# jason2714/de-i2i-gan

Measured on AMD Instinct MI355X. Metric: paired 256x256 images/sec (G+D train step), higher is better.
Workload: dtype bf16

## Files before the change

de-i2i-gan_amd/_lib.py:

```python
import ctypes
import os
from ctypes import POINTER, Structure, c_char_p, c_double, c_float, c_int, c_int64, c_size_t, c_void_p

_HERE = os.path.dirname(os.path.abspath(__file__))
LIB_PATH = os.path.join(_HERE, "lib", "libdei2i_hip.so")

BF16, F32 = 0, 1
ACT_NONE, ACT_RELU, ACT_LRELU = 0, 1, 2
PAD_ZERO, PAD_REFLECT = 0, 1
PROF_GATHER_GEMM, PROF_WGRAD, PROF_HALO_CONV, PROF_HALO_FOLD = 0, 1, 2, 3


class ConvDesc(Structure):
    _fields_ = [("dtype", c_int), ("N", c_int), ("H", c_int), ("W", c_int), ("Cin", c_int), ("Cout", c_int),
                ("CinS", c_int), ("CoutS", c_int), ("kh", c_int), ("kw", c_int), ("stride", c_int), ("pad", c_int),
                ("pad_mode", c_int), ("up", c_int)]


class ProDesc(Structure):
    _fields_ = [("A", c_void_p), ("B", c_void_p), ("n_stride", c_int), ("slope", c_float), ("ring", c_void_p)]


class EpiNormDesc(Structure):
    _fields_ = [("kind", c_int), ("up", c_int), ("act", c_int), ("group_images", c_int), ("x", c_void_p), ("mean", c_void_p),
# ... 86 lines not shown
    "dei2i_diffaug": (c_int, [c_int, c_int, c_int, c_int, c_int, c_int, c_int, c_int, _P, _P, _P, _P, _P]),
    "dei2i_prof_enable": (c_int, [c_int, c_int]),
    "dei2i_prof_collect": (c_int, [c_int, POINTER(c_int64), POINTER(c_double), POINTER(c_double)]),
    "dei2i_prof_collect_timed": (c_int, [c_int, POINTER(c_int64), POINTER(c_double)]),
    "dei2i_conv2d_fused_supported": (c_int, [_CD, c_int]),
    "dei2i_conv2d_stats_chunks": (c_int, [_CD]),
    "dei2i_conv2d_fwd_fused": (c_int, [_CD, _P, _P, _P, c_int, _P, _PD, _P, _P]),
    "dei2i_conv2d_wgrad_pro_supported": (c_int, [_CD]),
    "dei2i_conv2d_wgrad_oihw_pro": (c_int, [_CD, _P, _P, _P, c_size_t, _P, c_int, _PD, _P]),
    "dei2i_ring_pixels": (c_size_t, [c_int, c_int]),
    "dei2i_conv2d_ring_supported": (c_int, [_CD]),
    "dei2i_conv2d_dgrad_norm_supported": (c_int, [_CD]),
    "dei2i_conv2d_dgrad_norm_chunks": (c_int, [_CD]),
    "dei2i_conv2d_dgrad_input_norm": (c_int, [_CD, _P, _P, _P, _ED, _P]),
    "dei2i_in_act_bwd": (c_int, [c_int, c_int, c_int, c_int, c_int, _P, _P, _P, _P, c_float, _P, _P, _P, _P, _P, _P]),
    "dei2i_in_affine_act_bwd": (c_int, [c_int, c_int, c_int, c_int, c_int, _P, _P, _P, _P, c_float, _P, _P, _P, _P, _P, _P, _P]),
    "dei2i_avgpool2_fwd": (c_int, [c_int, c_int, c_int, c_int, c_int, _P, _P, _P]),
    "dei2i_avgpool2_bwd": (c_int, [c_int, c_int, c_int, c_int, c_int, _P, _P, _P]),
    "dei2i_spade_bwd_border": (c_int, [c_int, c_int, c_int, c_int, c_int, c_int, _P, _P, _P, _P, _P, _P, _P]),
    "dei2i_conv2d_fwd_ring": (c_int, [_CD, _P, _P, _P, _P, c_int, _P, _P, _P]),
    "dei2i_affine_act_img_fwd": (c_int, [c_int, c_int, c_int, c_int, _P, _P, _P, c_float, _P, _P]),
    "dei2i_spade_prep": (c_int, [c_int, c_int, c_int, c_int, c_int, c_int, _P, _P, c_int, c_float, _P, _P, _P, _P, _P, _P, _P]),
    "dei2i_affine_act_stats_fwd": (c_int, [c_int, c_int, c_int, c_int, c_int, _P, _P, _P, _P, c_int, _P, _P, _P]),
    "dei2i_launch_counts": (c_int, [POINTER(c_int64), c_int]),
    "dei2i_launch_counts_reset": (None, []),
    "dei2i_kernel_name": (c_char_p, [c_int]),
}

_lib = None


def load():
    global _lib
    if _lib is not None:
        return _lib
    import torch
    path = os.environ.get("DEI2I_LIB", LIB_PATH)
    if not os.path.exists(path):
        raise RuntimeError(
            f"libdei2i_hip.so not found at {path}: build it with `python -c 'import __graft_entry__ as g; g.build()'` "
            "(hipcc --offload-arch=gfx950).  There is no CPU / PyTorch fallback for the de-i2i-gan_amd ops.")
    lib = ctypes.CDLL(path)
    for name, (res, args) in SIGNATURES.items():
        fn = getattr(lib, name)
        fn.restype = res
        fn.argtypes = args
# ... 19 lines not shown
```

de-i2i-gan_amd/csrc/conv_api.hip:

```cpp
#include <hip/hip_runtime.h>

#include "../../include/dei2i_hip.h"
#include "launch.h"

namespace dei2i {

int g_use_wgrad_v2 = 1;
int g_use_wgrad_halo = 1;
int g_use_wgrad_thin = 1;
int g_dgrad_s2_ring = 1;
extern int g_halo16, g_halo16_fold;

static ConvShape to_shape(const dei2i_conv* c) {
  ConvShape s;
  s.N = c->N; s.H = c->H; s.W = c->W; s.Cin = c->Cin; s.Cout = c->Cout;
  s.kh = c->kh; s.kw = c->kw; s.stride = c->stride; s.pad = c->pad; s.pad_mode = c->pad_mode; s.up = c->up;
  return s;
}

static bool valid_conv(const dei2i_conv* c) {
  if (!c) return false;
  const int vec = c->dtype == DT_BF16 ? 8 : 4;
  if (c->dtype != DT_BF16 && c->dtype != DT_F32) return false;
  if (c->N <= 0 || c->H <= 0 || c->W <= 0 || c->Cin <= 0 || c->Cout <= 0) return false;
  if (c->CinS < c->Cin || c->CoutS < c->Cout || c->CinS % vec || c->CoutS % vec) return false;
  if (c->kh <= 0 || c->kw <= 0 || c->stride <= 0 || c->pad < 0 || c->up < 0 || c->up > 1) return false;
  if (c->kh < c->stride || c->kw < c->stride) return false;
  if (c->pad_mode == PAD_REFLECT && (c->pad >= (c->H << c->up) || c->pad >= (c->W << c->up))) return false;
  if (((c->H << c->up) + 2 * c->pad) < c->kh || ((c->W << c->up) + 2 * c->pad) < c->kw) return false;
  return true;
}

template <typename T>
// ... 74 lines not shown
    const int co = co0 + col, ci = ci0 + ch * VEC;
    if (co >= Cout || ci >= CinS) continue;
    float v[VEC];
#pragma unroll
    for (int e = 0; e < VEC; ++e) v[e] = tile[r * PT_ROW + ch * VEC + e];
    *reinterpret_cast<u32x4*>(fwd + ((size_t)co * taps + t) * CinS + ci) = Elem<T>::pack(v);
  }
  constexpr int DCH = PT_CO / VEC;
  for (int k = 0; k < pa.ncls; ++k) {
    const int th = pa.th[k], tw = pa.tw[k], nt = th * tw;
    T* dst = dgrad + pa.cls_begin[k];
    for (int i = threadIdx.x; i < PT_CI * nt * DCH; i += 256) {
      const int ch = i % DCH, r = i / DCH;
      const int t = r % nt, cil = r / nt;
      const int ci = ci0 + cil, co = co0 + ch * VEC;
      if (ci >= Cin || co >= CoutS) continue;
      const int jy = t / tw, jx = t - jy * tw;
      const int tap = (pa.ay[k] + s * jy) * kw + (pa.ax[k] + s * jx);
      float v[VEC];
#pragma unroll
      for (int e = 0; e < VEC; ++e) v[e] = tile[((ch * VEC + e) * taps + tap) * PT_ROW + cil];
      *reinterpret_cast<u32x4*>(dst + ((size_t)ci * nt + t) * CoutS + co) = Elem<T>::pack(v);
    }
  }
}

template <typename T>
__global__ void fold_pad_kernel(const T* __restrict__ ext, const T* __restrict__ addend, T* __restrict__ dx, int N, int H,
                                int W, int C, int pad, int reflect, int up) {
  constexpr int VEC = Elem<T>::VEC;
  const int Hl = H << up, Wl = W << up;
  const int off = reflect ? pad : 0;
  const int OH = Hl + 2 * off, OW = Wl + 2 * off;
  const int cv = C / VEC;
  const size_t total = (size_t)N * H * W * cv;
  for (size_t i = (size_t)blockIdx.x * blockDim.x + threadIdx.x; i < total; i += (size_t)gridDim.x * blockDim.x) {
    const int c = (int)(i % cv) * VEC;
    size_t r = i / cv;
    const int w = (int)(r % W); r /= W;
    const int h = (int)(r % H);
    const int n = (int)(r / H);
    float acc[VEC];
#pragma unroll
    for (int e = 0; e < VEC; ++e) acc[e] = 0.f;
    if (addend != nullptr) {
      float t[VEC];
// ... 272 lines not shown
    e = gather_gemm_multi(c->dtype, rows, wrows4, 4, dy, wd_packed, c->Cin, nullptr, ext_scratch, ws, ws_bytes, c->CinS, ACT_NONE, st, true);
    if (e != hipSuccess) return (int)e;
    const GatherDesc cols[4] = {sub_rect_desc(fr[0][0], 1, fr[0][0].Ho - 1, 0, 1), sub_rect_desc(fr[1][0], 0, fr[1][0].Ho - 1, 0, 1),
                                sub_rect_desc(fr[0][1], 1, fr[0][1].Ho - 1, fr[0][1].Wo - 1, 1),
                                sub_rect_desc(fr[1][1], 0, fr[1][1].Ho - 1, fr[1][1].Wo - 1, 1)};
    const long long wcols4[4] = {woff[0][0], woff[1][0], woff[0][1], woff[1][1]};
    e = gather_gemm_multi(c->dtype, cols, wcols4, 4, dy, wd_packed, c->Cin, nullptr, ext_scratch, ws, ws_bytes, c->CinS, ACT_NONE, st, true);
    if (e != hipSuccess) return (int)e;
    const int vec = c->dtype == DT_BF16 ? 8 : 4;
    const size_t total = (size_t)c->N * (2 * c->W + 2 * (c->H - 2)) * (c->CinS / vec);
    if (c->dtype == DT_BF16)
      hipLaunchKernelGGL(fold_border_kernel<bf16_t>, dim3(grid_for(total, 256)), dim3(256), 0, st, (const bf16_t*)ext_scratch, (bf16_t*)dx,
                         c->N, c->H, c->W, c->CinS, 1);
    else
      hipLaunchKernelGGL(fold_border_kernel<float>, dim3(grid_for(total, 256)), dim3(256), 0, st, (const float*)ext_scratch, (float*)dx, c->N,
                         c->H, c->W, c->CinS, 1);
    return (int)hipGetLastError();
  }
  const int rc = dei2i_conv2d_dgrad(c, dy, wd_packed, ext_scratch, ws, ws_bytes, s);
  if (rc != 0) return rc;
  return dei2i_fold_pad(c->dtype, c->N, c->H, c->W, c->CinS, c->pad, c->pad_mode, c->up, ext_scratch, nullptr, dx, s);
}

static bool dgrad_norm_shape_ok(const dei2i_conv* c) {
  if (!g_halo16 || !g_halo16_fold) return false;
  if (!valid_conv(c) || c->dtype != DT_BF16 || c->up) return false;
  if (c->kh != 3 || c->kw != 3 || c->stride != 1 || c->pad != 1 || c->pad_mode != PAD_REFLECT) return false;
  if (c->H % 16 != 0 || c->W % 32 != 0 || c->H < 32 || c->W < 64 || c->CinS < 64 || c->CinS % 8 != 0 || c->CoutS % 32 != 0) return false;
  if ((long long)c->N * c->H * c->W * c->CoutS >= (1ll << 31)) return false;
  const int tiles_m = c->N * (c->H / 16) * (c->W / 32);
  const int tn = c->CinS >= 128 ? (c->CinS + 127) / 128 : 1;
  return tiles_m * tn >= (num_cu() * 7) / 8;
}

int dei2i_conv2d_dgrad_norm_supported(const dei2i_conv* c) { return dgrad_norm_shape_ok(c) ? 1 : 0; }

int dei2i_conv2d_dgrad_norm_chunks(const dei2i_conv* c) { return (c->H / 16) * (c->W / 32); }

int dei2i_conv2d_dgrad_input_norm(const dei2i_conv* c, const void* dy, const void* wd_packed, void* dx, const dei2i_epi_norm* en,
                                  dei2i_stream s) {
  if (!dy || !wd_packed || !dx || !en || !dgrad_norm_shape_ok(c)) return DEI2I_ERR_BAD_ARG;
  if (!en->x || !en->mean || !en->rstd || !en->partial || en->up < 0 || en->up > 1) return DEI2I_ERR_BAD_ARG;
  const int kind = en->kind;
  if (kind == 1 ? !en->gb : (kind != 2 || !en->a || !en->b || en->up)) return DEI2I_ERR_BAD_ARG;
  if (en->group_images < 0 || (en->group_images > 0 && c->N % en->group_images != 0)) return DEI2I_ERR_BAD_ARG;
  ConvShape sh = to_shape(c);
// ... 151 lines not shown
```

de-i2i-gan_amd/csrc/geom.h:

```cpp
#pragma once
#include "common.h"

namespace dei2i {

struct GatherDesc {
  int N, Hs, Ws, Cs;
  int Clog;
  int Hl, Wl, up;
  int Ho, Wo, M;
  int sh, sw, by0, bx0;
  int th, tw, ys, xs;
  int pad_mode;
  int K;
  int wK, wtw, wty0, wtx0;
  int OH, OW, oys, oxs, oy0, ox0;
  int out_identity;
  FastDiv fd_cs, fd_tw, fd_wo, fd_howo;
};

inline void finish_desc(GatherDesc& g) {
  g.Hl = g.Hs << g.up;
  g.Wl = g.Ws << g.up;
  g.M = g.N * g.Ho * g.Wo;
  g.K = g.th * g.tw * g.Cs;
// ... 159 lines not shown
  int up;
  int act;
  int group_images;
};

DEI2I_HD long long packed_fwd_src(long long i, int Cin, int CinS, int taps) {
  const int ci = (int)(i % CinS);
  const long long r = i / CinS;
  const int t = (int)(r % taps);
  const long long co = r / taps;
  return ci < Cin ? (co * Cin + ci) * taps + t : -1;
}

DEI2I_HD long long packed_dgrad_src(long long i, int Cout, int Cin, int CoutS, int kh, int kw, int s, int ay, int ax,
                                    int th, int tw) {
  const int co = (int)(i % CoutS);
  const long long r = i / CoutS;
  const int t = (int)(r % (th * tw));
  const long long ci = r / (th * tw);
  const int jy = t / tw, jx = t - jy * tw;
  return co < Cout ? (((long long)co * Cin + ci) * kh + (ay + s * jy)) * kw + (ax + s * jx) : -1;
}

DEI2I_HD int fold_sources(int hs, int up, int Hl, int pad, int reflect, int* out) {
  const int off = reflect ? pad : 0;
  int n = 0;
  for (int a = 0; a < (1 << up); ++a) {
    const int hl = (hs << up) + a;
    out[n++] = hl + off;
    if (reflect) {
      if (hl >= 1 && hl <= pad) out[n++] = pad - hl;
      if (hl >= Hl - 1 - pad && hl <= Hl - 2) out[n++] = 2 * (Hl - 1) - hl + pad;
    }
  }
  return n;
}

}
```

de-i2i-gan_amd/csrc/reduce.hip:

```cpp
#include <hip/hip_runtime.h>
#include <math.h>

#include "../../include/dei2i_hip.h"
#include "launch.h"

namespace dei2i {

static inline int vec_of(int dtype) { return dtype == DT_BF16 ? 8 : 4; }

template <int NV, int VEC, typename OT = float>
DEI2I_D void block_combine_store(const float (&vals)[NV][VEC], int cv, int rpp, float* smem, OT* __restrict__ dst, int C) {
  const int tid = threadIdx.x;
  const int vcol = tid % cv, prow = tid / cv;
  __syncthreads();
  if (prow < rpp) {
#pragma unroll
    for (int q = 0; q < NV; ++q)
#pragma unroll
      for (int e = 0; e < VEC; ++e) smem[((q * VEC + e) * rpp + prow) * cv + vcol] = vals[q][e];
  }
  __syncthreads();
#pragma unroll 1
  for (int o = tid; o < NV * VEC * cv; o += 256) {
    const int qe = o / cv, vc = o - qe * cv;
// ... 311 lines not shown
        db[e] = g;
        v[0][e] += dxh;
        v[1][e] = fmaf(dxh, xh, v[1][e]);
      }
      if (gb_mode == 0) {
        *reinterpret_cast<u32x4*>(dgb_dense + q.opix * 2 * C + c) = Elem<T>::pack(dg);
        *reinterpret_cast<u32x4*>(dgb_dense + q.opix * 2 * C + C + c) = Elem<T>::pack(db);
      } else if (q.interior) {
#pragma unroll
        for (int e = 0; e < VEC; ++e) { v[2][e] += dg[e]; v[3][e] += db[e]; }
      }
    };
    int r = rbeg + prow;
    for (; r + rpp < rend; r += 2 * rpp) {
      const Row q0 = load(r), q1 = load(r + rpp);
      use(q0); use(q1);
    }
    if (r < rend) use(load(r));
  }
  block_combine_store<4, VEC>(v, cv, rpp, smem, partial + ((size_t)n * chunks + chunk) * 4 * C, C);
}

template <typename T>
__global__ __launch_bounds__(256) void spade_bwd_border_kernel(const T* __restrict__ dz, const T* __restrict__ x,
                                                               const float* __restrict__ mean, const float* __restrict__ rstd,
                                                               const T* __restrict__ gb, T* __restrict__ dgb_cls, int H,
                                                               int W, int C, int up, float slope = 0.f) {
  constexpr int VEC = Elem<T>::VEC;
  extern __shared__ float smem[];
  const int cls = blockIdx.x, n = blockIdx.y;
  const int cy = cls / 5, cx = cls - cy * 5;
  if (cy == 2 && cx == 2) return;
  const int cv = C / VEC, rpp = 256 / cv;
  const int tid = threadIdx.x, vcol = tid % cv, prow = tid / cv;
  const int Hs = H >> up, Ws = W >> up;
  const int y0 = cy < 2 ? cy : (cy == 2 ? 2 : H - 5 + cy), ny = cy == 2 ? H - 4 : 1;
  const int x0 = cx < 2 ? cx : (cx == 2 ? 2 : W - 5 + cx), nx = cx == 2 ? W - 4 : 1;
  const int count = ny * nx;
  float v[2][VEC];
#pragma unroll
  for (int e = 0; e < VEC; ++e) v[0][e] = v[1][e] = 0.f;
  if (prow < rpp) {
    const int c = vcol * VEC;
    float mv[VEC], rv[VEC], gm[VEC], bt[VEC];
    ldcoef<VEC>(mean + (size_t)n * C + c, mv);
    ldcoef<VEC>(rstd + (size_t)n * C + c, rv);
    const size_t gpix = ((size_t)n * 5 + cy) * 5 + cx;
    Elem<T>::unpack(*reinterpret_cast<const u32x4*>(gb + gpix * 2 * C + c), gm);
    Elem<T>::unpack(*reinterpret_cast<const u32x4*>(gb + gpix * 2 * C + C + c), bt);
    for (int i = prow; i < count; i += rpp) {
      const int h = y0 + i / nx, w = x0 + i % nx;
      const size_t opix = ((size_t)n * H + h) * W + w;
      float d[VEC], xv[VEC];
      Elem<T>::unpack(*reinterpret_cast<const u32x4*>(dz + opix * C + c), d);
      Elem<T>::unpack(*reinterpret_cast<const u32x4*>(x + (((size_t)n * Hs + (h >> up)) * Ws + (w >> up)) * C + c), xv);
#pragma unroll
      for (int e = 0; e < VEC; ++e) {
        const float xh = (xv[e] - mv[e]) * rv[e];
        const float g = fmaf(xh, 1.f + gm[e], bt[e]) > 0.f ? d[e] : slope * d[e];
        v[0][e] = fmaf(g, xh, v[0][e]);
        v[1][e] += g;
      }
    }
  }
  block_combine_store<2, VEC, T>(v, cv, rpp, smem, dgb_cls + (((size_t)n * 5 + cy) * 5 + cx) * 2 * C, C);
}

__global__ __launch_bounds__(256) void spade_bwd_finalize_kernel(const float* __restrict__ partial, int N, int chunks, int C,
                                                                 double count, float* __restrict__ coef,
                                                                 void* __restrict__ dgb_cls, int dtype) {
  const int c = blockIdx.x, n = blockIdx.y;
  double sq[4];
  combine_records<4>(partial, (size_t)n * chunks, chunks, C, c, sq);
  if (threadIdx.x != 0) return;
  coef[((size_t)n * 2 + 0) * C + c] = (float)(sq[0] / count);
  coef[((size_t)n * 2 + 1) * C + c] = (float)(sq[1] / count);
  if (dgb_cls != nullptr) {
// ... 34 lines not shown
    for (int e = 0; e < VEC; ++e) { acc[e] = 0.f; xh[e] = (xv[e] - mv[e]) * rv[e]; }
    for (int a = 0; a < (1 << up); ++a)
      for (int b = 0; b < (1 << up); ++b) {
        const int h = (hs << up) + a, w = (ws << up) + b;
        const size_t opix = ((size_t)n * H + h) * W + w;
        const size_t gpix = gb_mode == 0 ? opix : ((size_t)n * 5 + border_class(h, H)) * 5 + border_class(w, W);
        float d[VEC], gm[VEC], bt[VEC];
        Elem<T>::unpack(*reinterpret_cast<const u32x4*>(dz + opix * C + c), d);
        Elem<T>::unpack(*reinterpret_cast<const u32x4*>(gb + gpix * 2 * C + c), gm);
        Elem<T>::unpack(*reinterpret_cast<const u32x4*>(gb + gpix * 2 * C + C + c), bt);
#pragma unroll
        for (int e = 0; e < VEC; ++e) {
          const float g = fmaf(xh[e], 1.f + gm[e], bt[e]) > 0.f ? d[e] : slope * d[e];
          acc[e] = fmaf(g, 1.f + gm[e], acc[e]);
        }
      }
    float ad[VEC];
    if (addend != nullptr) Elem<T>::unpack(*reinterpret_cast<const u32x4*>(addend + i * VEC), ad);
    ldcoef<VEC>(coef + ((size_t)n * 2) * C + c, k1);
    ldcoef<VEC>(coef + ((size_t)n * 2 + 1) * C + c, k2);
#pragma unroll
    for (int e = 0; e < VEC; ++e) {
      float v = rv[e] * (acc[e] - cnt * k1[e] - cnt * xh[e] * k2[e]);
      if (addend != nullptr) v += ad[e];
      acc[e] = v;
    }
    *reinterpret_cast<u32x4*>(dx + i * VEC) = Elem<T>::pack(acc);
  }
}

template <typename T>
__global__ __launch_bounds__(256) void colsum_kernel(const T* __restrict__ g, float* __restrict__ partial, size_t rows, int C) {
  constexpr int VEC = Elem<T>::VEC;
  extern __shared__ float smem[];
  const int cv = C / VEC, rpp = 256 / cv;
  const int tid = threadIdx.x, vcol = tid % cv, prow = tid / cv;
  const size_t rows_per_block = (rows + gridDim.x - 1) / gridDim.x;
  const size_t rbeg = (size_t)blockIdx.x * rows_per_block;
  const size_t rend = rbeg + rows_per_block < rows ? rbeg + rows_per_block : rows;
  float v[1][VEC];
#pragma unroll
  for (int e = 0; e < VEC; ++e) v[0][e] = 0.f;
  if (prow < rpp) {
    const T* __restrict__ base = g + (size_t)vcol * VEC;
    auto acc = [&](const u32x4& q) {
      float f[VEC];
// ... 439 lines not shown
}

int dei2i_spade_bwd_apply(int dtype, int N, int H, int W, int C, int up, const void* dz, const void* x, const float* mean,
                          const float* rstd, const void* gb, int gb_mode, const float* partial, int chunks, void* dgb_cls,
                          float* coef, const void* addend, void* dx, dei2i_stream s) {
  const int vec = dtype == DT_BF16 ? 8 : 4;
  if (N <= 0 || H <= 0 || W <= 0 || !cv_ok(dtype, C) || up < 0 || up > 1 || !dz || !x || !mean || !rstd || !gb || !partial ||
      !coef || !dx)
    return DEI2I_ERR_BAD_ARG;
  hipStream_t st = (hipStream_t)s;
  hipLaunchKernelGGL(spade_bwd_finalize_kernel, dim3(C, N), dim3(combine_threads(chunks)), 0, st, partial, N, chunks, C,
                     (double)H * (double)W, coef, dgb_cls, dtype);
  const size_t total = (size_t)N * (H >> up) * (W >> up) * (C / vec);
  const unsigned grid = grid_for(total, 256, 256u * 16u);
  if (dtype == DT_BF16)
    hipLaunchKernelGGL(spade_bwd_apply_kernel<bf16_t>, dim3(grid), dim3(256), 0, st, (const bf16_t*)dz, (const bf16_t*)x, mean,
                       rstd, (const bf16_t*)gb, gb_mode, (const float*)coef, (const bf16_t*)addend, (bf16_t*)dx, N, H, W, C, up);
  else
    hipLaunchKernelGGL(spade_bwd_apply_kernel<float>, dim3(grid), dim3(256), 0, st, (const float*)dz, (const float*)x, mean,
                       rstd, (const float*)gb, gb_mode, (const float*)coef, (const float*)addend, (float*)dx, N, H, W, C, up);
  return (int)hipGetLastError();
}

int dei2i_in_act_bwd(int dtype, int N, int H, int W, int C, const void* dz, const void* x, const float* mean, const float* rstd,
                     float slope, const void* zero_table, float* partial, float* coef, const void* addend, void* dx, dei2i_stream s) {
  const int vec = dtype == DT_BF16 ? 8 : 4;
  if (N <= 0 || H < 4 || W < 4 || !cv_ok(dtype, C) || !dz || !x || !mean || !rstd || !zero_table || !partial || !coef || !dx)
    return DEI2I_ERR_BAD_ARG;
  hipStream_t st = (hipStream_t)s;
  const int chunks = dei2i_moments_chunks(H * W);
  if (dtype == DT_BF16)
    hipLaunchKernelGGL(spade_bwd_partial_kernel<bf16_t>, dim3(chunks, N), dim3(256), combine_lds(dtype, 4), st, (const bf16_t*)dz,
                       (const bf16_t*)x, mean, rstd, (const bf16_t*)zero_table, 1, (bf16_t*)nullptr, partial, H, W, C, 0, chunks, slope);
  else
    hipLaunchKernelGGL(spade_bwd_partial_kernel<float>, dim3(chunks, N), dim3(256), combine_lds(dtype, 4), st, (const float*)dz,
                       (const float*)x, mean, rstd, (const float*)zero_table, 1, (float*)nullptr, partial, H, W, C, 0, chunks, slope);
  hipLaunchKernelGGL(spade_bwd_finalize_kernel, dim3(C, N), dim3(combine_threads(chunks)), 0, st, (const float*)partial, N, chunks, C,
                     (double)H * (double)W, coef, (void*)nullptr, dtype);
  const size_t total = (size_t)N * H * W * (C / vec);
  const unsigned grid = grid_for(total, 256, 256u * 16u);
  if (dtype == DT_BF16)
    hipLaunchKernelGGL(spade_bwd_apply_kernel<bf16_t>, dim3(grid), dim3(256), 0, st, (const bf16_t*)dz, (const bf16_t*)x, mean, rstd,
                       (const bf16_t*)zero_table, 1, (const float*)coef, (const bf16_t*)addend, (bf16_t*)dx, N, H, W, C, 0, slope);
  else
    hipLaunchKernelGGL(spade_bwd_apply_kernel<float>, dim3(grid), dim3(256), 0, st, (const float*)dz, (const float*)x, mean, rstd,
                       (const float*)zero_table, 1, (const float*)coef, (const float*)addend, (float*)dx, N, H, W, C, 0, slope);
// ... 105 lines not shown
```

de-i2i-gan_amd/csrc/runtime.hip:

```cpp
#include <hip/hip_runtime.h>
#include <mutex>
#include <string>
#include <vector>

#include "../../include/dei2i_hip.h"
#include "launch.h"

namespace dei2i {

extern int g_use_wgrad_v2;
extern int g_use_wgrad_halo;
extern int g_use_wgrad_thin;
extern int g_dgrad_s2_ring;
extern int g_halo16, g_halo16_fold, g_halo16_s2;
static int g_cus = 256;
void set_num_cu_rt(int n) { g_cus = n > 0 ? n : 256; }
int num_cu() { return g_cus; }

struct ProfState {
  bool on = false;
  bool events = true;
  int every = 1;
  bool armed = false;
  double flops_timed = 0.0;
  size_t counted = 0;
  std::vector<hipEvent_t> starts, stops;
  size_t used = 0;
  double flops = 0.0;
};
static ProfState g_prof[PROF_FAMILIES];

static long long g_launches[K_COUNT];
void count_launch(int kid) { g_launches[kid]++; }
static const char* const g_kernel_names[K_COUNT] = {"gather_v1", "gather_v2", "halo_conv", "halo_conv_fp8", "thin_cin", "thin_cout",
                                                    "wgrad_v1", "wgrad_v2", "wgrad_halo", "wgrad_thin", "halo16_conv", "splitk_finalize", "halo16_s2"};

// ... 38 lines not shown
  set_num_cu(prop.multiProcessorCount);
  return 0;
}

const char* dei2i_error_string(int code) {
  if (code == DEI2I_ERR_BAD_ARG) return "dei2i: bad argument";
  if (code == DEI2I_ERR_WORKSPACE) return "dei2i: workspace too small";
  if (code >= 0) return hipGetErrorString((hipError_t)code);
  return "dei2i: unknown error";
}

int dei2i_set_option(const char* name, int value) {
  if (name == nullptr) return DEI2I_ERR_BAD_ARG;
  if (std::string(name) == "gather_gemm_v2") { set_use_v2(value); return 0; }
  if (std::string(name) == "wgrad_v2") { g_use_wgrad_v2 = value; return 0; }
  if (std::string(name) == "halo_conv") { set_use_halo(value); return 0; }
  if (std::string(name) == "thin_conv") { set_use_thin(value); return 0; }
  if (std::string(name) == "halo16") { g_halo16 = value; return 0; }
  if (std::string(name) == "halo16_fold") { g_halo16_fold = value; return 0; }
  if (std::string(name) == "halo16_s2") { g_halo16_s2 = value; return 0; }
  if (std::string(name) == "wgrad_halo") { g_use_wgrad_halo = value; return 0; }
  if (std::string(name) == "wgrad_thin") { g_use_wgrad_thin = value; return 0; }
  if (std::string(name) == "dgrad_s2_ring") { g_dgrad_s2_ring = value; return 0; }
  return DEI2I_ERR_BAD_ARG;
}

int dei2i_launch_counts(int64_t* out, int n) {
  for (int i = 0; i < n && i < K_COUNT; ++i) out[i] = (int64_t)g_launches[i];
  return K_COUNT;
}
void dei2i_launch_counts_reset(void) { for (int i = 0; i < K_COUNT; ++i) g_launches[i] = 0; }
const char* dei2i_kernel_name(int kid) { return kid >= 0 && kid < K_COUNT ? g_kernel_names[kid] : nullptr; }

int dei2i_prof_enable(int family, int on) {
  if (family < 0 || family >= PROF_FAMILIES) return DEI2I_ERR_BAD_ARG;
  ProfState& p = g_prof[family];
  p.on = on != 0;
  p.events = on != 2;
  p.every = on >= 3 ? on : 1;
  p.used = 0;
  p.counted = 0;
  p.flops = 0.0;
  p.flops_timed = 0.0;
  return 0;
}

// ... 31 lines not shown
```

de-i2i-gan_amd/ops.py:

```python
from __future__ import annotations

import ctypes
import weakref
from ctypes import byref, c_int, c_void_p
from dataclasses import dataclass
from typing import Optional

import torch

from . import _lib as L

ACT = {"none": L.ACT_NONE, None: L.ACT_NONE, "relu": L.ACT_RELU, "leaky_relu": L.ACT_LRELU}


@dataclass(frozen=True)
class Precision:
    name: str
    code: int
    dtype: torch.dtype
    vec: int

    def pad(self, c: int) -> int:
        return (c + self.vec - 1) // self.vec * self.vec

# ... 281 lines not shown


_descs = {}


def _desc(prec: Precision, g: ConvGeom, n: int, h: int, w: int, cins: int, couts: int) -> L.ConvDesc:
    key = (prec.code, g, n, h, w, cins, couts)
    d = _descs.get(key)
    if d is None:
        if len(_descs) > 4096:
            _descs.clear()
        d = _descs[key] = L.ConvDesc(prec.code, n, h, w, g.cin, g.cout, cins, couts, g.k, g.k, g.stride, g.pad,
                                     L.PAD_REFLECT if g.reflect else L.PAD_ZERO, 1 if g.up else 0)
    return d


class PackedWeights:

    def __init__(self):
        self._key = None
        self.fwd = None
        self.dgrad = None
        self.fp8 = None
        self._packed_on = None

    def _mark_packed(self):
        ev = self._packed_on[1] if self._packed_on is not None else torch.cuda.Event()
        ev.record()
        self._packed_on = (_stream_id(), ev, capture_serial)

    def _await_pack(self):
        if self._packed_on is not None and self._packed_on[0] != _stream_id():
            if self._packed_on[2] != capture_serial and torch.cuda.is_current_stream_capturing():
                return
            torch.cuda.current_stream().wait_event(self._packed_on[1])

    @staticmethod
    def _stamp(t: torch.Tensor):
        return (t.data_ptr(), t._version, getattr(t, "_dei2i_epoch", 0))

    def get(self, weight: torch.Tensor, sources, prec: Precision, geom: ConvGeom, cins: int, couts: int, need_dgrad: bool,
            need_fwd: bool = True, per_call: bool = False):
        key = ((), prec.code, cins, couts, self._stamp(weight)) if per_call else \
            (tuple(self._stamp(s) for s in sources), prec.code, cins, couts, None)
        if key == self._key and (self.fwd is not None or not need_fwd) and (self.dgrad is not None or not need_dgrad):
            self._await_pack()
            return self.fwd, self.dgrad
        lib = _lib_for(weight)
        if key != self._key:
            self._key, self.fwd, self.dgrad, self.fp8 = key, None, None, None
        d = _desc(prec, geom, 1, max(geom.k, 4), max(geom.k, 4), cins, couts)
        w = weight.detach()
        if w.dtype != torch.float32 or not w.is_contiguous():
            w = w.float().contiguous()
        self._await_pack()
        packed = False
        if need_fwd and need_dgrad and self.fwd is None and self.dgrad is None:
            self.fwd = torch.empty(lib.dei2i_packed_fwd_elems(byref(d)), dtype=prec.dtype, device=weight.device)
            self.dgrad = torch.empty(lib.dei2i_packed_dgrad_elems(byref(d)), dtype=prec.dtype, device=weight.device)
            L.check(lib.dei2i_pack_weight_both(byref(d), _p(w), _p(self.fwd), _p(self.dgrad), _stream()), "pack_weight_both")
            packed = True
        if need_fwd and self.fwd is None:
            self.fwd = torch.empty(lib.dei2i_packed_fwd_elems(byref(d)), dtype=prec.dtype, device=weight.device)
            L.check(lib.dei2i_pack_weight_fwd(byref(d), _p(w), _p(self.fwd), _stream()), "pack_weight_fwd")
            packed = True
        if need_dgrad and self.dgrad is None:
            self.dgrad = torch.empty(lib.dei2i_packed_dgrad_elems(byref(d)), dtype=prec.dtype, device=weight.device)
            L.check(lib.dei2i_pack_weight_dgrad(byref(d), _p(w), _p(self.dgrad), _stream()), "pack_weight_dgrad")
            packed = True
        if packed:
            self._mark_packed()
        return self.fwd, self.dgrad

    def get_fp8(self, weight: torch.Tensor, sources, prec: Precision, geom: ConvGeom, cins: int, couts: int):
        key = (tuple(self._stamp(s) for s in sources), prec.code, cins, couts, None)
        if key != self._key:
            self._key, self.fwd, self.dgrad, self.fp8 = key, None, None, None
        if self.fp8 is None:
            lib = _lib_for(weight)
            d = _desc(prec, geom, 1, 8, 32, cins, couts)
            w = weight.detach()
            if w.dtype != torch.float32 or not w.is_contiguous():
                w = w.float().contiguous()
            amax = torch.linalg.vector_norm(w, ord=float("inf")).reshape(1)
            wq = torch.empty(geom.cout * geom.k * geom.k * cins, dtype=torch.uint8, device=weight.device)
            dequant = torch.empty(1, dtype=torch.float32, device=weight.device)
            L.check(lib.dei2i_pack_weight_fwd_fp8(byref(d), _p(w), _p(amax), FP8_ACT_SCALE, _p(wq), _p(dequant), _stream()),
                    "pack_weight_fwd_fp8")
            self.fp8 = (wq, dequant)
        return self.fp8


_stats_stash = []


def _attach_stats(out):
    if _stats_stash:
        out._dei2i_stats = _stats_stash.pop()
    return out

# ... 756 lines not shown
        return (out, x_in) if skip else out

    @staticmethod
    def backward(ctx, dout, dskip=None):
        x, gb, mean, rstd = ctx.saved_tensors
        if dout is None:
            return dskip, None, None, None, None, None
        if dskip is not None:
            dskip = dskip.contiguous()
            if dskip.dtype != x.dtype or dskip.shape != x.shape:
                raise RuntimeError("spade_relu: identity-branch gradient does not match the activation")
        dx, dgb = _spade_backward(_lib_for(x), ctx.prec, dout, dskip, x, gb, mean, rstd, ctx.up, ctx.gb_mode, ctx.out_shape,
                                  hint=ctx.hint)
        return dx, dgb, None, None, None, None


def spade_relu(x, gb, up: bool, gb_mode: int, eps: float = 1e-5, skip: bool = False):
    del _fp8_stash[:]
    del _hint_stash[:]
    if skip:
        out, xs = _SpadeRelu.apply(x, gb, bool(up), int(gb_mode), float(eps), True)
        return _attach_hint(_attach_fp8(out)), xs
    return _attach_hint(_attach_fp8(_SpadeRelu.apply(x, gb, bool(up), int(gb_mode), float(eps))))


class _SpadeConv(torch.autograd.Function):

    @staticmethod
    def forward(ctx, x, gb, weight, up, eps, skip, cache: PackedWeights, sources, geom: ConvGeom, want_stats, ring_mode=False):
        prec = precision_of(x)
        x_in = x
        x, gb = x.contiguous(), gb.contiguous()
        if skip and (up or x is not x_in):
            raise ValueError("spade_conv(skip=True) wants a contiguous activation and no upsample")
        n, hs, ws, c = x.shape
        h, w = (hs * 2, ws * 2) if up else (hs, ws)
        lib = _lib_for(x)
        st = _stream()
        dev = x.device
        have = _stats_of(x, n, hs * ws, c)
        if have is not None:
            partial, chunks = have
        else:
            chunks = lib.dei2i_moments_chunks(hs * ws)
            partial = torch.empty((n, chunks, 2, c), dtype=torch.float32, device=dev)
            L.check(lib.dei2i_moments_partial(prec.code, n, hs * ws, c, _p(x), _p(partial), st), "moments_partial")
# ... 31 lines not shown

    @staticmethod
    def backward(ctx, dy, dskip=None):
        x, gb, coefs, ring, weight, z_src = ctx.saved_tensors
        prec, geom, up = ctx.prec, ctx.geom, ctx.up
        if dy is None:
            return (dskip,) + (None,) * 10
        lib = _lib_for(x)
        dy = dy.contiguous()
        n, h, w, c = ctx.out_shape
        if dskip is not None:
            dskip = dskip.contiguous()
            if dskip.dtype != x.dtype or dskip.shape != x.shape:
                raise RuntimeError("spade_conv: identity-branch gradient does not match the activation")
        dw = None
        if _wants_grad(ctx, 2):
            if ctx.ring_mode:
                dw = _conv_wgrad(lib, prec, geom, z_src, dy, weight, L.ProDesc(None, None, 0, 0.0, ring.data_ptr()), keep=(ring,))
            else:
                pro = L.ProDesc(coefs[2].data_ptr(), coefs[3].data_ptr(), c, 0.0, ring.data_ptr())
                dw = _conv_wgrad(lib, prec, geom, x, dy, weight, pro, keep=(coefs, ring))
        dx = dgb = None
        if _wants_grad(ctx, 0) or _wants_grad(ctx, 1):
            g_log = ConvGeom(geom.cin, geom.cout, geom.k, geom.stride, geom.pad, geom.reflect, False)
            hint = _NormBwdHint(1, x, coefs[0], coefs[1], gb=gb, up=up)
            dz = _conv_dgrad(lib, prec, g_log, (n, h, w, c), dy.shape[-1], dy, weight, ctx.cache, ctx.sources, ctx.per_call, x.dtype,
                             x.device, hint=hint)
            dx, dgb = _spade_backward(lib, prec, dz, dskip, x, gb, coefs[0], coefs[1], up, 1, ctx.out_shape, hint=hint)
        elif dskip is not None:
            dx = dskip
        return (dx, dgb, dw) + (None,) * 8


def spade_conv_supported(x, weight, geom: ConvGeom, need_grad: bool):
    if not (fuse_norm and x.is_cuda and x.dtype == torch.bfloat16 and not _fp8_forward):
        return None
    lib = _lib_for(x)
    n, hs, ws, c = x.shape
    d = _desc(BF16, geom, n, hs, ws, c, BF16.pad(geom.cout))
    wg_ok = (not need_grad) or bool(lib.dei2i_conv2d_wgrad_pro_supported(byref(d)))
    if fuse_pro and wg_ok and lib.dei2i_conv2d_fused_supported(byref(d), 1):
        return "pro"
    if fuse_ring and geom.up and wg_ok and lib.dei2i_conv2d_ring_supported(byref(d)):
        return "ring"
    return None

# ... 546 lines not shown
```

include/dei2i_hip.h:

```cpp
#ifndef DEI2I_HIP_H
#define DEI2I_HIP_H

#include <stddef.h>
#include <stdint.h>

#ifdef __cplusplus
extern "C" {
#endif

typedef void* dei2i_stream;

#define DEI2I_BF16 0
#define DEI2I_F32 1
#define DEI2I_ACT_NONE 0
#define DEI2I_ACT_RELU 1
#define DEI2I_ACT_LRELU 2
#define DEI2I_PAD_ZERO 0
#define DEI2I_PAD_REFLECT 1

#define DEI2I_ERR_BAD_ARG (-2)
#define DEI2I_ERR_WORKSPACE (-3)

typedef struct dei2i_conv {
  int dtype;
// ... 171 lines not shown
int dei2i_conv2d_wgrad_pro_supported(const dei2i_conv* c);
int dei2i_conv2d_wgrad_oihw_pro(const dei2i_conv* c, const void* x, const void* dy, float* scratch, size_t scratch_elems,
                                float* dw_oihw, int accumulate, const dei2i_pro* pro, dei2i_stream s);
int dei2i_conv2d_ring_supported(const dei2i_conv* c);
int dei2i_conv2d_fwd_ring(const dei2i_conv* c, const void* z_src, const void* ring, const void* w_packed, const float* bias, int act,
                          void* y, float* stats, dei2i_stream s);
typedef struct dei2i_epi_norm {
  int kind;
  int up;
  int act;
  int group_images;
  const void* x;
  const float* mean;
  const float* rstd;
  const void* gb;
  const float* a;
  const float* b;
  float* partial;
} dei2i_epi_norm;
int dei2i_conv2d_dgrad_norm_supported(const dei2i_conv* c);
int dei2i_conv2d_dgrad_norm_chunks(const dei2i_conv* c);
int dei2i_conv2d_dgrad_input_norm(const dei2i_conv* c, const void* dy, const void* wd_packed, void* dx, const dei2i_epi_norm* en,
                                  dei2i_stream s);
int dei2i_in_act_bwd(int dtype, int N, int H, int W, int C, const void* dz, const void* x, const float* mean, const float* rstd,
                     float slope, const void* zero_table, float* partial, float* coef, const void* addend, void* dx, dei2i_stream s);
int dei2i_in_affine_act_bwd(int dtype, int N, int H, int W, int C, const void* dz, const void* x, const float* mean,
                            const float* rstd, float slope, const void* gb_table, void* dgb_table, float* partial, float* coef,
                            const void* addend, void* dx, dei2i_stream s);
int dei2i_avgpool2_fwd(int dtype, int N, int H, int W, int C, const void* x, void* out, dei2i_stream s);
int dei2i_avgpool2_bwd(int dtype, int N, int H, int W, int C, const void* dout, void* dx, dei2i_stream s);
int dei2i_spade_bwd_border(int dtype, int N, int H, int W, int C, int up, const void* dz, const void* x, const float* mean,
                           const float* rstd, const void* gb, void* dgb_cls, dei2i_stream s);
int dei2i_affine_act_img_fwd(int dtype, int N, int HW, int C, const void* x, const float* A, const float* B, float slope, void* out,
                             dei2i_stream s);
size_t dei2i_ring_pixels(int H, int W);
int dei2i_spade_prep(int dtype, int N, int Hs, int Ws, int C, int up, const void* x, const float* partial, int chunks, float eps,
                     const void* gb_table, float* mean, float* rstd, float* A, float* B, void* ring, dei2i_stream s);

int dei2i_launch_counts(int64_t* out, int n);
void dei2i_launch_counts_reset(void);
const char* dei2i_kernel_name(int kid);

#ifdef __cplusplus
}
#endif
#endif
// ... 1 lines not shown
```

Baseline: 463.0.

## Compute upsample-conv input gradient as stride-2 4x4 conv on cells with fused SPADE backward

After: 469.8 (median of 6 runs). +1.5%, better.

```diff
diff --git a/de-i2i-gan_amd/_lib.py b/de-i2i-gan_amd/_lib.py
--- a/de-i2i-gan_amd/_lib.py
+++ b/de-i2i-gan_amd/_lib.py
@@ -132,6 +132,12 @@
     "dei2i_affine_act_img_fwd": (c_int, [c_int, c_int, c_int, c_int, _P, _P, _P, c_float, _P, _P]),
     "dei2i_spade_prep": (c_int, [c_int, c_int, c_int, c_int, c_int, c_int, _P, _P, c_int, c_float, _P, _P, _P, _P, _P, _P, _P]),
     "dei2i_affine_act_stats_fwd": (c_int, [c_int, c_int, c_int, c_int, c_int, _P, _P, _P, _P, c_int, _P, _P, _P]),
+    "dei2i_upcell_taps": (c_int, [c_int, POINTER(c_int)]),
+    "dei2i_packed_upcells_elems": (c_size_t, [_CD]),
+    "dei2i_pack_weight_upcells": (c_int, [_CD, _P, _P, _P]),
+    "dei2i_conv2d_upcells_supported": (c_int, [_CD]),
+    "dei2i_conv2d_dgrad_up_cells": (c_int, [_CD, _P, _P, _P, _P, _P, _P, c_size_t, _P]),
+    "dei2i_spade_bwd_cells": (c_int, [c_int, c_int, c_int, c_int, c_int, _P, _P, _P, _P, _P, _P, _P, _P, _P, _P, _P, _P]),
     "dei2i_launch_counts": (c_int, [POINTER(c_int64), c_int]),
     "dei2i_launch_counts_reset": (None, []),
     "dei2i_kernel_name": (c_char_p, [c_int]),
diff --git a/de-i2i-gan_amd/csrc/conv_api.hip b/de-i2i-gan_amd/csrc/conv_api.hip
--- a/de-i2i-gan_amd/csrc/conv_api.hip
+++ b/de-i2i-gan_amd/csrc/conv_api.hip
@@ -9,6 +9,7 @@
 int g_use_wgrad_halo = 1;
 int g_use_wgrad_thin = 1;
 int g_dgrad_s2_ring = 1;
+int g_upconv_cells = 1;
 extern int g_halo16, g_halo16_fold;
 
 static ConvShape to_shape(const dei2i_conv* c) {
@@ -129,6 +130,18 @@
       for (int e = 0; e < VEC; ++e) v[e] = tile[((ch * VEC + e) * taps + tap) * PT_ROW + cil];
       *reinterpret_cast<u32x4*>(dst + ((size_t)ci * nt + t) * CoutS + co) = Elem<T>::pack(v);
     }
+  }
+}
+
+template <typename T>
+__global__ void pack_upcells_kernel(const float* __restrict__ w, T* __restrict__ dst, int Cout, int Cin, int CoutS) {
+  const long long total = (long long)Cin * 16 * CoutS;
+  for (long long i = (long long)blockIdx.x * blockDim.x + threadIdx.x; i < total; i += (long long)gridDim.x * blockDim.x) {
+    long long src[4];
+    const int n = packed_upcell_srcs(i, Cout, Cin, CoutS, src);
+    float e = 0.f;
+    for (int k = 0; k < n; ++k) e += w[src[k]];
+    Elem<T>::store(dst + i, e);
   }
 }
 
@@ -447,6 +460,56 @@
   return dei2i_fold_pad(c->dtype, c->N, c->H, c->W, c->CinS, c->pad, c->pad_mode, c->up, ext_scratch, nullptr, dx, s);
 }
 
+static bool upcells_shape(const dei2i_conv* c, dei2i_conv* vc) {
+  if (!valid_conv(c) || c->dtype != DT_BF16 || !c->up) return false;
+  if (c->kh != 3 || c->kw != 3 || c->stride != 1 || c->pad != 1 || c->pad_mode != PAD_REFLECT) return false;
+  if (c->H < 4 || c->W < 4) return false;
+  if ((long long)c->N * (2 * c->H + 2) * (2 * c->W + 2) * (c->CinS > c->CoutS ? c->CinS : c->CoutS) >= (1ll << 31)) return false;
+  *vc = *c;
+  vc->H = 2 * c->H; vc->W = 2 * c->W; vc->Cin = c->Cout; vc->Cout = c->Cin; vc->CinS = c->CoutS; vc->CoutS = c->CinS;
+  vc->kh = vc->kw = 4; vc->stride = 2; vc->pad = 1; vc->pad_mode = PAD_ZERO; vc->up = 0;
+  return valid_conv(vc);
+}
+
+int dei2i_upcell_taps(int u, int* k0) {
+  int k = 0;
+  const int n = (u >= 0 && u < 4) ? upcell_taps(u, &k) : 0;
+  if (k0) *k0 = k;
+  return n;
+}
+
+size_t dei2i_packed_upcells_elems(const dei2i_conv* c) { return (size_t)c->Cin * 16 * c->CoutS; }
+
+int dei2i_pack_weight_upcells(const dei2i_conv* c, const float* w, void* packed, dei2i_stream s) {
+  dei2i_conv vc;
+  if (!c || !w || !packed || !upcells_shape(c, &vc)) return DEI2I_ERR_BAD_ARG;
+  const unsigned grid = grid_for(dei2i_packed_upcells_elems(c), 256);
+  hipLaunchKernelGGL(pack_upcells_kernel<bf16_t>, dim3(grid), dim3(256), 0, (hipStream_t)s, w, (bf16_t*)packed, c->Cout, c->Cin, c->CoutS);
+  return (int)hipGetLastError();
+}
+
+int dei2i_conv2d_upcells_supported(const dei2i_conv* c) {
+  dei2i_conv vc;
+  if (!c || g_upconv_cells == 0 || !upcells_shape(c, &vc)) return 0;
+  return (g_upconv_cells >= 2 || (size_t)c->N * 4 * c->H * c->W * c->CinS >= ((size_t)48 << 20)) ? 1 : 0;
+}
+
+int dei2i_conv2d_dgrad_up_cells(const dei2i_conv* c, const void* dy, const void* we_packed, const void* wd_packed, void* dz_cells,
+                                void* frame_ext, float* ws, size_t ws_bytes, dei2i_stream s) {
+  dei2i_conv vc;
+  if (!c || !dy || !we_packed || !wd_packed || !dz_cells || !frame_ext || !upcells_shape(c, &vc)) return DEI2I_ERR_BAD_ARG;
+  const int rc = dei2i_conv2d_fwd(&vc, dy, we_packed, nullptr, ACT_NONE, dz_cells, ws, ws_bytes, s);
+  if (rc != 0) return rc;
+  ConvShape sh = to_shape(c);
+  sh.H = 2 * c->H; sh.W = 2 * c->W; sh.up = 0;
+  const GatherDesc fr = make_dgrad_desc(sh, c->CoutS, 0, 0);
+  const GatherDesc rect[4] = {sub_rect_desc(fr, 0, 3, 0, fr.OW), sub_rect_desc(fr, fr.OH - 3, 3, 0, fr.OW),
+                              sub_rect_desc(fr, 3, fr.OH - 6, 0, 3), sub_rect_desc(fr, 3, fr.OH - 6, fr.OW - 3, 3)};
+  const long long woffs[4] = {0, 0, 0, 0};
+  return (int)gather_gemm_multi(c->dtype, rect, woffs, 4, dy, wd_packed, c->Cin, nullptr, frame_ext, ws, ws_bytes, c->CinS, ACT_NONE,
+                                (hipStream_t)s, true);
+}
+
 static bool dgrad_norm_shape_ok(const dei2i_conv* c) {
   if (!g_halo16 || !g_halo16_fold) return false;
   if (!valid_conv(c) || c->dtype != DT_BF16 || c->up) return false;
diff --git a/de-i2i-gan_amd/csrc/geom.h b/de-i2i-gan_amd/csrc/geom.h
--- a/de-i2i-gan_amd/csrc/geom.h
+++ b/de-i2i-gan_amd/csrc/geom.h
@@ -205,6 +205,24 @@
   return co < Cout ? (((long long)co * Cin + ci) * kh + (ay + s * jy)) * kw + (ax + s * jx) : -1;
 }
 
+DEI2I_HD int upcell_taps(int u, int* k0) {
+  *k0 = u == 0 ? 2 : (u == 1 ? 1 : 0);
+  return (u == 1 || u == 2) ? 2 : 1;
+}
+
+DEI2I_HD int packed_upcell_srcs(long long i, int Cout, int Cin, int CoutS, long long* src) {
+  const int co = (int)(i % CoutS);
+  const long long r = i / CoutS;
+  const int t = (int)(r % 16);
+  const long long ci = r / 16;
+  if (co >= Cout) return 0;
+  int ky0, kx0, n = 0;
+  const int ny = upcell_taps(t >> 2, &ky0), nx = upcell_taps(t & 3, &kx0);
+  for (int a = 0; a < ny; ++a)
+    for (int b = 0; b < nx; ++b) src[n++] = (((long long)co * Cin + ci) * 3 + (ky0 + a)) * 3 + (kx0 + b);
+  return n;
+}
+
 DEI2I_HD int fold_sources(int hs, int up, int Hl, int pad, int reflect, int* out) {
   const int off = reflect ? pad : 0;
   int n = 0;
diff --git a/de-i2i-gan_amd/csrc/reduce.hip b/de-i2i-gan_amd/csrc/reduce.hip
--- a/de-i2i-gan_amd/csrc/reduce.hip
+++ b/de-i2i-gan_amd/csrc/reduce.hip
@@ -357,6 +357,22 @@
 }
 
 template <typename T>
+DEI2I_D void load_frame_px(const T* __restrict__ ext, int n, int h, int w, int H, int W, int C, int c, float (&d)[Elem<T>::VEC]) {
+  constexpr int VEC = Elem<T>::VEC;
+  int ys[6], xs[6];
+  const int ny = fold_sources(h, 0, H, 1, 1, ys), nx = fold_sources(w, 0, W, 1, 1, xs);
+#pragma unroll
+  for (int e = 0; e < VEC; ++e) d[e] = 0.f;
+  for (int a = 0; a < ny; ++a)
+    for (int b = 0; b < nx; ++b) {
+      float t[VEC];
+      Elem<T>::unpack(*reinterpret_cast<const u32x4*>(ext + (((size_t)n * (H + 2) + ys[a]) * (W + 2) + xs[b]) * C + c), t);
+#pragma unroll
+      for (int e = 0; e < VEC; ++e) d[e] += t[e];
+    }
+}
+
+template <typename T, bool FRAME = false>
 __global__ __launch_bounds__(256) void spade_bwd_border_kernel(const T* __restrict__ dz, const T* __restrict__ x,
                                                                const float* __restrict__ mean, const float* __restrict__ rstd,
                                                                const T* __restrict__ gb, T* __restrict__ dgb_cls, int H,
@@ -387,7 +403,8 @@
       const int h = y0 + i / nx, w = x0 + i % nx;
       const size_t opix = ((size_t)n * H + h) * W + w;
       float d[VEC], xv[VEC];
-      Elem<T>::unpack(*reinterpret_cast<const u32x4*>(dz + opix * C + c), d);
+      if constexpr (FRAME) load_frame_px<T>(dz, n, h, w, H, W, C, c, d);
+      else Elem<T>::unpack(*reinterpret_cast<const u32x4*>(dz + opix * C + c), d);
       Elem<T>::unpack(*reinterpret_cast<const u32x4*>(x + (((size_t)n * Hs + (h >> up)) * Ws + (w >> up)) * C + c), xv);
 #pragma unroll
       for (int e = 0; e < VEC; ++e) {
@@ -468,6 +485,116 @@
 #pragma unroll
     for (int e = 0; e < VEC; ++e) {
       float v = rv[e] * (acc[e] - cnt * k1[e] - cnt * xh[e] * k2[e]);
+      if (addend != nullptr) v += ad[e];
+      acc[e] = v;
+    }
+    *reinterpret_cast<u32x4*>(dx + i * VEC) = Elem<T>::pack(acc);
+  }
+}
+
+template <typename T>
+DEI2I_D void spade_cell_dxhat(const T* __restrict__ dzc, const T* __restrict__ ext, const T* __restrict__ gb, int n, int hs, int ws,
+                              int Hs, int Ws, int C, int c, const float (&xh)[Elem<T>::VEC], float (&dxh)[Elem<T>::VEC],
+                              float (&gsum)[Elem<T>::VEC]) {
+  constexpr int VEC = Elem<T>::VEC;
+  const int H = 2 * Hs, W = 2 * Ws;
+#pragma unroll
+  for (int e = 0; e < VEC; ++e) dxh[e] = gsum[e] = 0.f;
+  auto add = [&](const float (&d)[VEC], size_t gpix) {
+    float gm[VEC], bt[VEC];
+    Elem<T>::unpack(*reinterpret_cast<const u32x4*>(gb + gpix * 2 * C + c), gm);
+    Elem<T>::unpack(*reinterpret_cast<const u32x4*>(gb + gpix * 2 * C + C + c), bt);
+#pragma unroll
+    for (int e = 0; e < VEC; ++e) {
+      const float g = fmaf(xh[e], 1.f + gm[e], bt[e]) > 0.f ? d[e] : 0.f;
+      dxh[e] = fmaf(g, 1.f + gm[e], dxh[e]);
+      gsum[e] += g;
+    }
+  };
+  float d[VEC];
+  if (hs >= 1 && hs < Hs - 1 && ws >= 1 && ws < Ws - 1) {
+    Elem<T>::unpack(*reinterpret_cast<const u32x4*>(dzc + (((size_t)n * Hs + hs) * Ws + ws) * C + c), d);
+    add(d, ((size_t)n * 5 + 2) * 5 + 2);
+  } else {
+    for (int a = 0; a < 2; ++a)
+      for (int b = 0; b < 2; ++b) {
+        const int h = 2 * hs + a, w = 2 * ws + b;
+        load_frame_px<T>(ext, n, h, w, H, W, C, c, d);
+        add(d, ((size_t)n * 5 + border_class(h, H)) * 5 + border_class(w, W));
+      }
+  }
+}
+
+template <typename T>
+__global__ __launch_bounds__(256) void spade_bwd_partial_cells_kernel(const T* __restrict__ dzc, const T* __restrict__ ext,
+                                                                      const T* __restrict__ x, const float* __restrict__ mean,
+                                                                      const float* __restrict__ rstd, const T* __restrict__ gb,
+                                                                      float* __restrict__ partial, int Hs, int Ws, int C, int chunks) {
+  constexpr int VEC = Elem<T>::VEC;
+  extern __shared__ float smem[];
+  const int cv = C / VEC, rpp = 256 / cv;
+  const int tid = threadIdx.x, vcol = tid % cv, prow = tid / cv;
+  const int chunk = blockIdx.x, n = blockIdx.y;
+  const int HW = Hs * Ws;
+  const int rows_per_chunk = (HW + chunks - 1) / chunks;
+  const int rbeg = chunk * rows_per_chunk, rend = min(HW, rbeg + rows_per_chunk);
+  float v[4][VEC];
+#pragma unroll
+  for (int q = 0; q < 4; ++q)
+#pragma unroll
+    for (int e = 0; e < VEC; ++e) v[q][e] = 0.f;
+  if (prow < rpp) {
+    const int c = vcol * VEC;
+    float mv[VEC], rv[VEC];
+    ldcoef<VEC>(mean + (size_t)n * C + c, mv);
+    ldcoef<VEC>(rstd + (size_t)n * C + c, rv);
+    for (int r = rbeg + prow; r < rend; r += rpp) {
+      const int hs = r / Ws, ws = r - hs * Ws;
+      float xv[VEC], xh[VEC], dxh[VEC], gs[VEC];
+      Elem<T>::unpack(*reinterpret_cast<const u32x4*>(x + ((size_t)n * HW + r) * C + c), xv);
+#pragma unroll
+      for (int e = 0; e < VEC; ++e) xh[e] = (xv[e] - mv[e]) * rv[e];
+      spade_cell_dxhat<T>(dzc, ext, gb, n, hs, ws, Hs, Ws, C, c, xh, dxh, gs);
+      const bool interior = hs >= 1 && hs < Hs - 1 && ws >= 1 && ws < Ws - 1;
+#pragma unroll
+      for (int e = 0; e < VEC; ++e) {
+        v[0][e] += dxh[e];
+        v[1][e] = fmaf(dxh[e], xh[e], v[1][e]);
+        if (interior) { v[2][e] = fmaf(gs[e], xh[e], v[2][e]); v[3][e] += gs[e]; }
+      }
+    }
+  }
+  block_combine_store<4, VEC>(v, cv, rpp, smem, partial + ((size_t)n * chunks + chunk) * 4 * C, C);
+}
+
+template <typename T>
+__global__ void spade_bwd_apply_cells_kernel(const T* __restrict__ dzc, const T* __restrict__ ext, const T* __restrict__ x,
+                                             const float* __restrict__ mean, const float* __restrict__ rstd,
+                                             const T* __restrict__ gb, const float* __restrict__ coef,
+                                             const T* __restrict__ addend, T* __restrict__ dx, int N, int Hs, int Ws, int C) {
+  constexpr int VEC = Elem<T>::VEC;
+  const int cv = C / VEC;
+  const size_t total = (size_t)N * Hs * Ws * cv;
+  for (size_t i = (size_t)blockIdx.x * blockDim.x + threadIdx.x; i < total; i += (size_t)gridDim.x * blockDim.x) {
+    const int c = (int)(i % cv) * VEC;
+    size_t r = i / cv;
+    const int ws = (int)(r % Ws); r /= Ws;
+    const int hs = (int)(r % Hs);
+    const int n = (int)(r / Hs);
+    float acc[VEC], gs[VEC], xv[VEC], xh[VEC], mv[VEC], rv[VEC], k1[VEC], k2[VEC];
+    ldcoef<VEC>(mean + (size_t)n * C + c, mv);
+    ldcoef<VEC>(rstd + (size_t)n * C + c, rv);
+    Elem<T>::unpack(*reinterpret_cast<const u32x4*>(x + i * VEC), xv);
+#pragma unroll
+    for (int e = 0; e < VEC; ++e) xh[e] = (xv[e] - mv[e]) * rv[e];
+    spade_cell_dxhat<T>(dzc, ext, gb, n, hs, ws, Hs, Ws, C, c, xh, acc, gs);
+    float ad[VEC];
+    if (addend != nullptr) Elem<T>::unpack(*reinterpret_cast<const u32x4*>(addend + i * VEC), ad);
+    ldcoef<VEC>(coef + ((size_t)n * 2) * C + c, k1);
+    ldcoef<VEC>(coef + ((size_t)n * 2 + 1) * C + c, k2);
+#pragma unroll
+    for (int e = 0; e < VEC; ++e) {
+      float v = rv[e] * (acc[e] - 4.f * k1[e] - 4.f * xh[e] * k2[e]);
       if (addend != nullptr) v += ad[e];
       acc[e] = v;
     }
@@ -953,6 +1080,27 @@
   return (int)hipGetLastError();
 }
 
+int dei2i_spade_bwd_cells(int dtype, int N, int Hs, int Ws, int C, const void* dzc, const void* ext, const void* x, const float* mean,
+                          const float* rstd, const void* gb, float* partial, void* dgb_cls, float* coef, const void* addend, void* dx,
+                          dei2i_stream s) {
+  if (dtype != DT_BF16 || N <= 0 || Hs < 4 || Ws < 4 || !cv_ok(dtype, C) || !dzc || !ext || !x || !mean || !rstd || !gb || !partial ||
+      !dgb_cls || !coef || !dx)
+    return DEI2I_ERR_BAD_ARG;
+  hipStream_t st = (hipStream_t)s;
+  const bf16_t *dc = (const bf16_t*)dzc, *ex = (const bf16_t*)ext, *xs = (const bf16_t*)x, *g = (const bf16_t*)gb;
+  const int chunks = dei2i_moments_chunks(Hs * Ws);
+  hipLaunchKernelGGL((spade_bwd_border_kernel<bf16_t, true>), dim3(25, N), dim3(256), combine_lds(dtype, 2), st, ex, xs, mean, rstd, g,
+                     (bf16_t*)dgb_cls, 2 * Hs, 2 * Ws, C, 1);
+  hipLaunchKernelGGL(spade_bwd_partial_cells_kernel<bf16_t>, dim3(chunks, N), dim3(256), combine_lds(dtype, 4), st, dc, ex, xs, mean,
+                     rstd, g, partial, Hs, Ws, C, chunks);
+  hipLaunchKernelGGL(spade_bwd_finalize_kernel, dim3(C, N), dim3(combine_threads(chunks)), 0, st, (const float*)partial, N, chunks, C,
+                     4.0 * (double)Hs * (double)Ws, coef, dgb_cls, dtype);
+  const size_t total = (size_t)N * Hs * Ws * (C / 8);
+  hipLaunchKernelGGL(spade_bwd_apply_cells_kernel<bf16_t>, dim3(grid_for(total, 256, 256u * 16u)), dim3(256), 0, st, dc, ex, xs, mean,
+                     rstd, g, (const float*)coef, (const bf16_t*)addend, (bf16_t*)dx, N, Hs, Ws, C);
+  return (int)hipGetLastError();
+}
+
 int dei2i_in_act_bwd(int dtype, int N, int H, int W, int C, const void* dz, const void* x, const float* mean, const float* rstd,
                      float slope, const void* zero_table, float* partial, float* coef, const void* addend, void* dx, dei2i_stream s) {
   const int vec = dtype == DT_BF16 ? 8 : 4;
diff --git a/de-i2i-gan_amd/csrc/runtime.hip b/de-i2i-gan_amd/csrc/runtime.hip
--- a/de-i2i-gan_amd/csrc/runtime.hip
+++ b/de-i2i-gan_amd/csrc/runtime.hip
@@ -12,6 +12,7 @@
 extern int g_use_wgrad_halo;
 extern int g_use_wgrad_thin;
 extern int g_dgrad_s2_ring;
+extern int g_upconv_cells;
 extern int g_halo16, g_halo16_fold, g_halo16_s2;
 static int g_cus = 256;
 void set_num_cu_rt(int n) { g_cus = n > 0 ? n : 256; }
@@ -96,6 +97,7 @@
   if (std::string(name) == "wgrad_halo") { g_use_wgrad_halo = value; return 0; }
   if (std::string(name) == "wgrad_thin") { g_use_wgrad_thin = value; return 0; }
   if (std::string(name) == "dgrad_s2_ring") { g_dgrad_s2_ring = value; return 0; }
+  if (std::string(name) == "upconv_cells") { g_upconv_cells = value; return 0; }
   return DEI2I_ERR_BAD_ARG;
 }
 
diff --git a/de-i2i-gan_amd/ops.py b/de-i2i-gan_amd/ops.py
--- a/de-i2i-gan_amd/ops.py
+++ b/de-i2i-gan_amd/ops.py
@@ -327,6 +327,7 @@
         self.fwd = None
         self.dgrad = None
         self.fp8 = None
+        self.upcells = None
         self._packed_on = None
 
     def _mark_packed(self):
@@ -353,7 +354,7 @@
             return self.fwd, self.dgrad
         lib = _lib_for(weight)
         if key != self._key:
-            self._key, self.fwd, self.dgrad, self.fp8 = key, None, None, None
+            self._key, self.fwd, self.dgrad, self.fp8, self.upcells = key, None, None, None, None
         d = _desc(prec, geom, 1, max(geom.k, 4), max(geom.k, 4), cins, couts)
         w = weight.detach()
         if w.dtype != torch.float32 or not w.is_contiguous():
@@ -377,10 +378,27 @@
             self._mark_packed()
         return self.fwd, self.dgrad
 
+    def get_upcells(self, weight: torch.Tensor, sources, prec: Precision, geom: ConvGeom, cins: int, couts: int, per_call: bool = False):
+        key = ((), prec.code, cins, couts, self._stamp(weight)) if per_call else \
+            (tuple(self._stamp(s) for s in sources), prec.code, cins, couts, None)
+        if key != self._key:
+            self._key, self.fwd, self.dgrad, self.fp8, self.upcells = key, None, None, None, None
+        self._await_pack()
+        if self.upcells is None:
+            lib = _lib_for(weight)
+            d = _desc(prec, geom, 1, 4, 4, cins, couts)
+            w = weight.detach()
+            if w.dtype != torch.float32 or not w.is_contiguous():
+                w = w.float().contiguous()
+            self.upcells = torch.empty(lib.dei2i_packed_upcells_elems(byref(d)), dtype=prec.dtype, device=weight.device)
+            L.check(lib.dei2i_pack_weight_upcells(byref(d), _p(w), _p(self.upcells), _stream()), "pack_weight_upcells")
+            self._mark_packed()
+        return self.upcells
+
     def get_fp8(self, weight: torch.Tensor, sources, prec: Precision, geom: ConvGeom, cins: int, couts: int):
         key = (tuple(self._stamp(s) for s in sources), prec.code, cins, couts, None)
         if key != self._key:
-            self._key, self.fwd, self.dgrad, self.fp8 = key, None, None, None
+            self._key, self.fwd, self.dgrad, self.fp8, self.upcells = key, None, None, None, None
         if self.fp8 is None:
             lib = _lib_for(weight)
             d = _desc(prec, geom, 1, 8, 32, cins, couts)
@@ -1183,6 +1201,28 @@
         out, xs = _SpadeRelu.apply(x, gb, bool(up), int(gb_mode), float(eps), True)
         return _attach_hint(_attach_fp8(out)), xs
     return _attach_hint(_attach_fp8(_SpadeRelu.apply(x, gb, bool(up), int(gb_mode), float(eps))))
+
+
+def _spade_conv_backward_cells(lib, ctx, d, dy, dskip, x, gb, coefs, weight):
+    prec, geom = ctx.prec, ctx.geom
+    n, hs, ws, c = x.shape
+    couts = dy.shape[-1]
+    dev = x.device
+    _, wd = ctx.cache.get(weight, ctx.sources, prec, geom, c, couts, need_dgrad=True, need_fwd=False, per_call=ctx.per_call)
+    we = ctx.cache.get_upcells(weight, ctx.sources, prec, geom, c, couts, per_call=ctx.per_call)
+    g_log = _desc(prec, ConvGeom(geom.cin, geom.cout, geom.k, geom.stride, geom.pad, geom.reflect, False), n, 2 * hs, 2 * ws, c, couts)
+    wsp = _workspace(dev, lib.dei2i_conv2d_workspace_bytes(byref(g_log)))
+    ext = _workspace(dev, n * (2 * hs + 2) * (2 * ws + 2) * c * x.element_size(), slot="dgrad_frame")
+    dzc = torch.empty_like(x)
+    L.check(lib.dei2i_conv2d_dgrad_up_cells(byref(d), _p(dy), _p(we), _p(wd), _p(dzc), _p(ext), _p(wsp), wsp.numel() * 4, _stream()),
+            "conv2d_dgrad_up_cells")
+    partial = torch.empty((n, lib.dei2i_moments_chunks(hs * ws), 4, c), dtype=torch.float32, device=dev)
+    coef = torch.empty((n, 2, c), dtype=torch.float32, device=dev)
+    dgb = torch.empty_like(gb)
+    dx = torch.empty_like(x)
+    L.check(lib.dei2i_spade_bwd_cells(prec.code, n, hs, ws, c, _p(dzc), _p(ext), _p(x), _p(coefs[0]), _p(coefs[1]), _p(gb), _p(partial),
+                                      _p(dgb), _p(coef), _p(dskip), _p(dx), _stream()), "spade_bwd_cells")
+    return dx, dgb
 
 
 class _SpadeConv(torch.autograd.Function):
@@ -1260,6 +1300,10 @@
                 dw = _conv_wgrad(lib, prec, geom, x, dy, weight, pro, keep=(coefs, ring))
         dx = dgb = None
         if _wants_grad(ctx, 0) or _wants_grad(ctx, 1):
+            d_up = _desc(prec, geom, n, x.shape[1], x.shape[2], c, dy.shape[-1])
+            if up and prec is BF16 and lib.dei2i_conv2d_upcells_supported(byref(d_up)):
+                dx, dgb = _spade_conv_backward_cells(lib, ctx, d_up, dy, dskip, x, gb, coefs, weight)
+                return (dx, dgb, dw) + (None,) * 8
             g_log = ConvGeom(geom.cin, geom.cout, geom.k, geom.stride, geom.pad, geom.reflect, False)
             hint = _NormBwdHint(1, x, coefs[0], coefs[1], gb=gb, up=up)
             dz = _conv_dgrad(lib, prec, g_log, (n, h, w, c), dy.shape[-1], dy, weight, ctx.cache, ctx.sources, ctx.per_call, x.dtype,
diff --git a/include/dei2i_hip.h b/include/dei2i_hip.h
--- a/include/dei2i_hip.h
+++ b/include/dei2i_hip.h
@@ -217,6 +217,15 @@
 int dei2i_conv2d_dgrad_norm_chunks(const dei2i_conv* c);
 int dei2i_conv2d_dgrad_input_norm(const dei2i_conv* c, const void* dy, const void* wd_packed, void* dx, const dei2i_epi_norm* en,
                                   dei2i_stream s);
+int dei2i_upcell_taps(int u, int* k0);
+size_t dei2i_packed_upcells_elems(const dei2i_conv* c);
+int dei2i_pack_weight_upcells(const dei2i_conv* c, const float* w_oihw, void* packed, dei2i_stream s);
+int dei2i_conv2d_upcells_supported(const dei2i_conv* c);
+int dei2i_conv2d_dgrad_up_cells(const dei2i_conv* c, const void* dy, const void* we_packed, const void* wd_packed, void* dz_cells,
+                                void* frame_ext, float* ws, size_t ws_bytes, dei2i_stream s);
+int dei2i_spade_bwd_cells(int dtype, int N, int Hs, int Ws, int C, const void* dz_cells, const void* frame_ext, const void* x,
+                          const float* mean, const float* rstd, const void* gb, float* partial, void* dgb_cls, float* coef,
+                          const void* addend, void* dx, dei2i_stream s);
 int dei2i_in_act_bwd(int dtype, int N, int H, int W, int C, const void* dz, const void* x, const float* mean, const float* rstd,
                      float slope, const void* zero_table, float* partial, float* coef, const void* addend, void* dx, dei2i_stream s);
 int dei2i_in_affine_act_bwd(int dtype, int N, int H, int W, int C, const void* dz, const void* x, const float* mean,
```
